# huawei-noah/xingtian

Measured on NVIDIA H100. Metric: learner env-steps/sec (Atari 84x84x4 PPO), higher is better.
Workload: dtype f32 (bf16x3 split on wgmma, fp32 accumulate in registers)

## Files before the change

### xingtian_b200/csrc/optim.cuh

```cuda
#pragma once
#include <cuda_bf16.h>
#include <cuda_runtime.h>
#include <stdint.h>

#include "bp_gemm.cuh"
#include "launch.cuh"

namespace xtb {

constexpr int OPT_CHUNK = 1024;
constexpr int OPT_THREADS = 256;

struct AdamState {
  float beta1_pow, beta2_pow, lr_t, grad_norm;
  unsigned int iterations;
};
struct AdamHyper {
  float lr, beta1, beta2, eps, clip;
  float decay;
};

__device__ __forceinline__ void adam_prep(AdamState* st, const AdamHyper* hyp, double* norm_sq, float* seg_scale, int n_seg,
                                          int clip_mode, float grad_scale) {
  const float clip = hyp->clip, beta1 = hyp->beta1, beta2 = hyp->beta2;
  float lr = hyp->lr;
  if (hyp->decay != 0.f) lr = lr / (1.f + hyp->decay * (float)st->iterations);
  st->iterations += 1;
  double tot = 0.0;
  for (int s = 0; s < n_seg; s++) tot += norm_sq[s];
  float gs = fabsf(grad_scale);
  float gnorm = (float)sqrt(tot) * gs;
  st->grad_norm = gnorm;
  if (clip_mode == 1) {
    float sc = clip / fmaxf(gnorm, clip);
    for (int s = 0; s < n_seg; s++) seg_scale[s] = sc * grad_scale;
  } else if (clip_mode == 2) {
    for (int s = 0; s < n_seg; s++) {
      float n = (float)sqrt(norm_sq[s]) * gs;
      seg_scale[s] = (n > clip ? clip / n : 1.f) * grad_scale;
    }
  } else {
    for (int s = 0; s < n_seg; s++) seg_scale[s] = grad_scale;
  }
  for (int s = 0; s < n_seg; s++) norm_sq[s] = 0.0;
  float b1p = st->beta1_pow * beta1, b2p = st->beta2_pow * beta2;
  st->beta1_pow = b1p; st->beta2_pow = b2p;
  st->lr_t = lr * sqrtf(1.f - b2p) / (1.f - b1p);
}

constexpr int SQN_GROUP = 4;
__global__ void __launch_bounds__(OPT_THREADS)
sqnorm_kernel(const float* __restrict__ g, const int* __restrict__ blk_seg,
              const long long* __restrict__ blk_beg, const int* __restrict__ blk_len, int n_blk,
              double* __restrict__ norm_sq, unsigned int* __restrict__ ticket, AdamState* st, const AdamHyper* __restrict__ hyp,
              float* seg_scale, int n_seg, int clip_mode, float grad_scale) {
  pdl_wait(); pdl_trigger();
  __shared__ float red[OPT_THREADS / 32];
  auto flush = [&](float s, int seg) {
#pragma unroll
    for (int o = 16; o > 0; o >>= 1) s += __shfl_xor_sync(0xffffffffu, s, o);
    if ((threadIdx.x & 31) == 0) red[threadIdx.x >> 5] = s;
    __syncthreads();
    if (threadIdx.x < 32) {
      float t = threadIdx.x < OPT_THREADS / 32 ? red[threadIdx.x] : 0.f;
#pragma unroll
      for (int o = 16; o > 0; o >>= 1) t += __shfl_xor_sync(0xffffffffu, t, o);
      if (threadIdx.x == 0) atomicAdd(norm_sq + seg, (double)t);
    }
    __syncthreads();
  };
  const int e0 = blockIdx.x * SQN_GROUP, e1 = min(e0 + SQN_GROUP, n_blk);
  float s = 0.f;
  int cur = blk_seg[e0];
  for (int e = e0; e < e1; e++) {
    if (blk_seg[e] != cur) { flush(s, cur); s = 0.f; cur = blk_seg[e]; }
    const float* p = g + blk_beg[e];
    const int n = blk_len[e];
    if ((blk_beg[e] & 3) == 0) {
      const int nv = n & ~3;
      for (int i = threadIdx.x * 4; i < nv; i += OPT_THREADS * 4) {
        const float4 v = *reinterpret_cast<const float4*>(p + i);
        s = fmaf(v.x, v.x, s); s = fmaf(v.y, v.y, s); s = fmaf(v.z, v.z, s); s = fmaf(v.w, v.w, s);
      }
      for (int i = nv + threadIdx.x; i < n; i += OPT_THREADS) { float v = p[i]; s = fmaf(v, v, s); }
    } else {
      for (int i = threadIdx.x; i < n; i += OPT_THREADS) { float v = p[i]; s = fmaf(v, v, s); }
    }
  }
  flush(s, cur);
  if (threadIdx.x == 0) {
    __threadfence();
    if (atomicAdd(ticket, 1u) == gridDim.x - 1) {
      __threadfence();
      *ticket = 0;
      adam_prep(st, hyp, norm_sq, seg_scale, n_seg, clip_mode, grad_scale);
    }
  }
}

__global__ void __launch_bounds__(OPT_THREADS)
adam_kernel(float* __restrict__ p, const float* __restrict__ g, float* __restrict__ m,
            float* __restrict__ v, const int* __restrict__ blk_seg,
            const long long* __restrict__ blk_beg, const int* __restrict__ blk_len,
            const float* __restrict__ seg_scale, const AdamState* __restrict__ st, const AdamHyper* __restrict__ hyp,
            const bp::BlobSeg* __restrict__ bsegs, int n_bsegs, __nv_bfloat16* __restrict__ w_hi, long long w_lo_off) {
  pdl_wait(); pdl_trigger();
  const float beta1 = hyp->beta1, beta2 = hyp->beta2, eps = hyp->eps;
  long long beg = blk_beg[blockIdx.x];
  int n = blk_len[blockIdx.x];
  float sc = seg_scale[blk_seg[blockIdx.x]];
  float lr_t = st->lr_t;
  const bool vec = ((beg & 3) == 0);
  int nv = vec ? (n & ~3) : 0;
  for (int i = threadIdx.x * 4; i < nv; i += OPT_THREADS * 4) {
    long long j = beg + i;
    float4 g4 = *reinterpret_cast<const float4*>(g + j);
    float4 m4 = *reinterpret_cast<const float4*>(m + j);
    float4 v4 = *reinterpret_cast<const float4*>(v + j);
    float4 p4 = *reinterpret_cast<const float4*>(p + j);
    float gg[4] = {g4.x * sc, g4.y * sc, g4.z * sc, g4.w * sc};
    float mm[4] = {m4.x, m4.y, m4.z, m4.w}, vv[4] = {v4.x, v4.y, v4.z, v4.w}, pp[4] = {p4.x, p4.y, p4.z, p4.w};
#pragma unroll
    for (int q = 0; q < 4; q++) {
      mm[q] = beta1 * mm[q] + (1.f - beta1) * gg[q];
      vv[q] = beta2 * vv[q] + (1.f - beta2) * gg[q] * gg[q];
      pp[q] -= lr_t * mm[q] / (sqrtf(vv[q]) + eps);
    }
    *reinterpret_cast<float4*>(m + j) = make_float4(mm[0], mm[1], mm[2], mm[3]);
    *reinterpret_cast<float4*>(v + j) = make_float4(vv[0], vv[1], vv[2], vv[3]);
    *reinterpret_cast<float4*>(p + j) = make_float4(pp[0], pp[1], pp[2], pp[3]);
    if (w_hi) bp::blob_store4(bsegs, n_bsegs, w_hi, w_lo_off, j, pp);
  }
  for (int i = nv + threadIdx.x; i < n; i += OPT_THREADS) {
    long long j = beg + i;
    float gg = g[j] * sc;
    float mm = beta1 * m[j] + (1.f - beta1) * gg;
    float vv = beta2 * v[j] + (1.f - beta2) * gg * gg;
    m[j] = mm; v[j] = vv;
    float pn = p[j] - lr_t * mm / (sqrtf(vv) + eps);
    p[j] = pn;
    if (w_hi) bp::blob_store1(bsegs, n_bsegs, w_hi, w_lo_off, j, pn);
  }
}

template <bool CENTRED>
__global__ void __launch_bounds__(OPT_THREADS)
rmsprop_kernel(float* __restrict__ p, const float* __restrict__ g, float* __restrict__ ms, float* __restrict__ mg,
               const int* __restrict__ blk_seg, const long long* __restrict__ blk_beg, const int* __restrict__ blk_len,
               const float* __restrict__ seg_scale, const AdamHyper* __restrict__ hyp, float rho, float rms_eps,
               const bp::BlobSeg* __restrict__ bsegs, int n_bsegs, __nv_bfloat16* __restrict__ w_hi, long long w_lo_off) {
  pdl_wait(); pdl_trigger();
  const long long beg = blk_beg[blockIdx.x];
  const int n = blk_len[blockIdx.x];
  const float sc = seg_scale[blk_seg[blockIdx.x]], lr = hyp->lr;
  const bool vec = ((beg & 3) == 0);
  const int nv = vec ? (n & ~3) : 0;
  for (int i = threadIdx.x * 4; i < nv; i += OPT_THREADS * 4) {
    const long long j = beg + i;
    const float4 g4 = *reinterpret_cast<const float4*>(g + j);
    const float4 s4 = *reinterpret_cast<const float4*>(ms + j);
    const float4 a4 = CENTRED ? *reinterpret_cast<const float4*>(mg + j) : make_float4(0.f, 0.f, 0.f, 0.f);
    const float4 p4 = *reinterpret_cast<const float4*>(p + j);
    float gg[4] = {g4.x * sc, g4.y * sc, g4.z * sc, g4.w * sc};
    float ss[4] = {s4.x, s4.y, s4.z, s4.w}, aa[4] = {a4.x, a4.y, a4.z, a4.w}, pp[4] = {p4.x, p4.y, p4.z, p4.w};
#pragma unroll
    for (int q = 0; q < 4; q++) {
      ss[q] = rho * ss[q] + (1.f - rho) * gg[q] * gg[q];
      if (CENTRED) {
        aa[q] = rho * aa[q] + (1.f - rho) * gg[q];
        pp[q] -= lr * gg[q] / sqrtf(ss[q] - aa[q] * aa[q] + rms_eps);
      } else {
        pp[q] -= lr * gg[q] / sqrtf(ss[q] + rms_eps);
      }
    }
    *reinterpret_cast<float4*>(ms + j) = make_float4(ss[0], ss[1], ss[2], ss[3]);
    if (CENTRED) *reinterpret_cast<float4*>(mg + j) = make_float4(aa[0], aa[1], aa[2], aa[3]);
    *reinterpret_cast<float4*>(p + j) = make_float4(pp[0], pp[1], pp[2], pp[3]);
    if (w_hi) bp::blob_store4(bsegs, n_bsegs, w_hi, w_lo_off, j, pp);
  }
  for (int i = nv + threadIdx.x; i < n; i += OPT_THREADS) {
    const long long j = beg + i;
    const float gg = g[j] * sc;
    const float ss = rho * ms[j] + (1.f - rho) * gg * gg;
    ms[j] = ss;
    float pn;
    if (CENTRED) {
      const float aa = rho * mg[j] + (1.f - rho) * gg;
      mg[j] = aa;
      pn = p[j] - lr * gg / sqrtf(ss - aa * aa + rms_eps);
    } else {
      pn = p[j] - lr * gg / sqrtf(ss + rms_eps);
    }
    p[j] = pn;
    if (w_hi) bp::blob_store1(bsegs, n_bsegs, w_hi, w_lo_off, j, pn);
  }
}

}
```

### xingtian_b200/csrc/xtb_engine.cu

```cuda
#include "../../include/xtb200.h"

#include <cuda_runtime.h>

#include <atomic>
#include <cmath>
#include <cstdarg>
#include <cstdio>
#include <cstring>
#include <map>
#include <memory>
#include <string>
#include <tuple>
#include <vector>

#include "gemm_f32.cuh"
#include "optim.cuh"
#include "rl_kernels.cuh"
#include "qmix.cuh"
#include "scc.cuh"
#include "stager.cuh"
#include "bp_gemm.cuh"
#include "comm.cuh"
#include <cstdlib>
#include <type_traits>
// ... 1320 lines not shown
      rc = comm_fork_allreduce(comm, net->grads + early_off, early_cnt, st);
      if (rc) return rc;
    }
    if (lp.d.kind == XTB_DUELING) {
      const int s = lp.d.src, s2 = lp.d.k;
      rc = op_dgrad(net, i, written[s] ? 1 : 0, batch, st, false, written[s2] ? 1 : 0);
      if (rc) return rc;
      written[s] = written[s2] = 1; has_grad[s] = has_grad[s2] = 1;
    } else if (lp.d.src != 0) {
      int s = lp.d.src;
      rc = op_dgrad(net, i, written[s] ? 1 : 0, batch, st, fuse_bias[s] == 1);
      if (rc) return rc;
      written[s] = 1; has_grad[s] = 1; dy[s] = 1;
    }
  }
  if (o.dobs) {
    bool first = true;
    for (int i = 0; i < nl; i++) {
      const LayerPlan& lp = net->L[i];
      if (lp.d.src != 0 || lp.d.kind != XTB_DENSE || (o.skip & (1u << i))) continue;
      if (!has_grad[i + 1]) continue;
      int rc = ensure_f32(net, i + 1, batch, true, st);
      if (rc) return rc;
      ADense<float> al{(const float*)gout_f32(net, i + 1), nullptr, lp.N};
      BTransposed bl{net->params + lp.w_off, lp.N};
      EpiDgrad ep{o.dobs, o.dobs, 0, lp.K, first ? 0 : 1, nullptr, 0};
      launch_gemm(al, bl, ep, batch, lp.K, lp.N, false, st);
      LAUNCH_CHECK();
      first = false;
    }
    if (first) CUDA_TRY(cudaMemsetAsync(o.dobs, 0, (size_t)batch * net->tsize[0] * sizeof(float), st));
  }
  int rc = flush_reductions(net, st);
  if (rc || !comm || comm->world == 1) return rc;
  if (early_cnt == 0) return xtb_comm_allreduce(comm, net->grads, net->n_params, stream);
  int nrc = g_nccl.GroupStart();
  if (!nrc && early_off > 0) nrc = g_nccl.AllReduce(net->grads, net->grads, (size_t)early_off, kNcclFloat, kNcclSum, comm->comm, st);
  const long long tail = net->n_params - (early_off + early_cnt);
  if (!nrc && tail > 0)
    nrc = g_nccl.AllReduce(net->grads + early_off + early_cnt, net->grads + early_off + early_cnt, (size_t)tail, kNcclFloat, kNcclSum, comm->comm, st);
  int erc = g_nccl.GroupEnd();
  if (nrc || erc) return fail(XTB_ERR_CUDA, "ncclAllReduce: %s", g_nccl.GetErrorString(nrc ? nrc : erc));
  return comm_join(comm, st);
}

extern "C" int xtb_net_bench_layer(xtb_net* net, int layer, int which, const void* obs, const int32_t* gather_idx,
                                   int batch, void* stream) {
  if (!net || !net->ws || !net->grads) return fail(XTB_ERR_STATE, "xtb_net_bench_layer: net not bound");
  if (layer < 0 || layer >= (int)net->L.size() || batch <= 0 || batch > net->max_batch) return fail(XTB_ERR_ARG, "bad layer/batch");
  cudaStream_t st = S(stream);
  for (int t = 1; t <= (int)net->L.size(); t++)
    for (bool grad : {false, true})
      if (forms(net, t, grad) == kNone) wrote(net, t, grad, kF32);
  if (which == 0) return op_forward(net, layer, net->params, true, obs, gather_idx, batch, batch, false, st);
  if (which == 1) { int rc = op_wgrad(net, layer, obs, gather_idx, batch, st, true); net->pending.clear(); return rc; }
  if (which == 2) {
    if (net->L[layer].d.src == 0) return fail(XTB_ERR_ARG, "layer reads the observation: no data gradient");
    int rc = op_dgrad(net, layer, 0, batch, st);
    net->pending.clear();
    return rc;
  }
  if (which == 3) { wrote(net, 0, false, kNone); return op_decode(net, obs, gather_idx, batch, st); }
  return fail(XTB_ERR_ARG, "xtb_net_bench_layer: which must be 0..3");
}


extern "C" int xtb_categorical_sample(const float* logits, int batch, int adim, const float* uniforms,
                                      uint64_t seed, uint64_t offset, int32_t* action, float* logp, void* stream) {
  if (!logits || !action || !logp || batch <= 0 || adim <= 0) return fail(XTB_ERR_ARG, "xtb_categorical_sample: bad argument");
  XLAUNCH(sample_kernel<Categorical>, (batch + 127) / 128, 128, 0, S(stream), logits, (const float*)nullptr, batch, batch, adim,
          uniforms, seed, offset, (const unsigned long long*)nullptr, 0, action, logp, (const float*)nullptr, (float*)nullptr);
  LAUNCH_CHECK();
  return XTB_OK;
}

extern "C" int xtb_argmax(const float* q, int batch, int adim, int32_t* action, void* stream) {
  if (!q || !action || batch <= 0 || adim <= 0) return fail(XTB_ERR_ARG, "xtb_argmax: bad argument");
  XLAUNCH(argmax_kernel, (batch + 127) / 128, 128, 0, S(stream), q, batch, adim, action);
  LAUNCH_CHECK();
  return XTB_OK;
}

extern "C" int xtb_gae(const float* value, const float* reward, const uint8_t* done, int n_env, int n_step,
                       float gamma, float lam, int sign_clip, float* adv, float* old_value, float* target_value,
                       void* stream) {
  if (!value || !reward || !done || !adv || !old_value || !target_value) return fail(XTB_ERR_ARG, "xtb_gae: null pointer");
  if (n_env == 0 || n_step == 0) return XTB_OK;
  if (n_env < 0 || n_step < 0) return fail(XTB_ERR_ARG, "xtb_gae: negative size");
  int threads = 128;
  int blocks = (n_env * 32 + threads - 1) / threads;
  XLAUNCH(gae_kernel, blocks, threads, 0, S(stream), value, reward, done, n_env, n_step, gamma, lam, sign_clip, adv,
                                                old_value, target_value);
  LAUNCH_CHECK();
  return XTB_OK;
}

extern "C" int xtb_ppo_loss_grad(const float* logits, const float* v, const int32_t* gather_idx,
                                 const int32_t* action, const float* old_logp, const float* adv,
                                 const float* old_v, const float* target_v, int batch, int adim,
                                 const xtb_ppo_hyper* hp, float inv_count, float* dlogits, float* dv,
                                 float* loss_out, void* stream) {
  if (!logits || !v || !action || !old_logp || !adv || !old_v || !target_v || !hp || !dlogits || !dv || !loss_out)
    return fail(XTB_ERR_ARG, "xtb_ppo_loss_grad: null pointer");
  if (batch <= 0 || adim <= 0 || adim > MAX_ADIM) return fail(XTB_ERR_ARG, "xtb_ppo_loss_grad: batch/adim out of range");
  PpoHyperDev h{hp->clip_ratio, hp->ent_coef, hp->vf_clip, hp->critic_coef};
  XLAUNCH(ppo_loss_kernel, (batch + 127) / 128, 128, 0, S(stream), logits, v, gather_idx, action, old_logp, adv, old_v,
                                                              target_v, batch, adim, h, inv_count, dlogits, dv, loss_out);
  LAUNCH_CHECK();
  return XTB_OK;
}

extern "C" int xtb_diag_gaussian_sample(const float* mean, const float* log_std, int batch, int adim, const float* normals,
                                        uint64_t seed, uint64_t offset, float* action, float* logp, void* stream) {
  if (!mean || !log_std || !action || !logp || batch <= 0 || adim <= 0 || adim > MAX_ADIM)
    return fail(XTB_ERR_ARG, "xtb_diag_gaussian_sample: bad argument");
  XLAUNCH(sample_kernel<DiagGaussian>, (batch + 127) / 128, 128, 0, S(stream), mean, log_std, batch, batch, adim, normals, seed,
          offset, (const unsigned long long*)nullptr, 0, action, logp, (const float*)nullptr, (float*)nullptr);
  LAUNCH_CHECK();
  return XTB_OK;
}

extern "C" int xtb_ppo_gauss_loss_grad(const float* mean, const float* v, const float* log_std, const int32_t* gather_idx,
                                       const float* action, const float* old_logp, const float* adv, const float* old_v,
                                       const float* target_v, int batch, int adim, const xtb_ppo_hyper* hp, float inv_count,
                                       float* dmean, float* dv, float* dlog_std, float* loss_out, void* stream) {
  if (!mean || !v || !log_std || !action || !old_logp || !adv || !old_v || !target_v || !hp || !dmean || !dv || !dlog_std || !loss_out)
    return fail(XTB_ERR_ARG, "xtb_ppo_gauss_loss_grad: null pointer");
  if (batch <= 0 || adim <= 0 || adim > MAX_ADIM) return fail(XTB_ERR_ARG, "xtb_ppo_gauss_loss_grad: batch/adim out of range");
  PpoHyperDev h{hp->clip_ratio, hp->ent_coef, hp->vf_clip, hp->critic_coef};
  if (adim <= 8)
    XLAUNCH(ppo_gauss_loss_kernel<8>, 1, GAUSS_LOSS_THREADS, 0, S(stream), mean, v, log_std, gather_idx, action, old_logp, adv, old_v,
            target_v, batch, adim, h, inv_count, dmean, dv, dlog_std, loss_out);
  else
    XLAUNCH(ppo_gauss_loss_kernel<MAX_ADIM>, 1, GAUSS_LOSS_THREADS, 0, S(stream), mean, v, log_std, gather_idx, action, old_logp, adv,
            old_v, target_v, batch, adim, h, inv_count, dmean, dv, dlog_std, loss_out);
  LAUNCH_CHECK();
  return XTB_OK;
}

extern "C" int xtb_vtrace_loss_grad(const float* tp_logits, const float* baseline, const float* bp_logits,
                                    const int32_t* action, const uint8_t* done, const float* reward,
                                    int n_traj, int step_len, int adim, float gamma, float* dlogits,
                                    float* dbaseline, float* vs_out, float* pg_adv_out, float* loss_out,
                                    void* stream) {
  if (!tp_logits || !baseline || !bp_logits || !action || !done || !reward || !dlogits || !dbaseline || !loss_out)
    return fail(XTB_ERR_ARG, "xtb_vtrace_loss_grad: null pointer");
  if (n_traj <= 0 || step_len < 2 || adim <= 0 || adim > MAX_ADIM) return fail(XTB_ERR_ARG, "xtb_vtrace_loss_grad: bad sizes");
  int threads = 128;
  int blocks = (n_traj * 32 + threads - 1) / threads;
  XLAUNCH(vtrace_kernel, blocks, threads, 0, S(stream), tp_logits, baseline, bp_logits, action, done, reward, n_traj,
                                                   step_len, adim, gamma, dlogits, dbaseline, vs_out, pg_adv_out, loss_out);
  LAUNCH_CHECK();
  return XTB_OK;
}

extern "C" int xtb_dqn_td_loss_grad(const float* q, const float* q_next_target, const float* q_next_online, const int32_t* idx,
                                    const int32_t* action, const float* reward, const uint8_t* done, const float* disc, int batch,
                                    int adim, float gamma, float huber_delta, float inv_count, float* dq, float* y_out,
                                    float* loss_out, void* stream) {
  if (!q || !q_next_target || !action || !reward || !done || !dq || !loss_out) return fail(XTB_ERR_ARG, "xtb_dqn_td_loss_grad: null pointer");
  if (batch <= 0 || adim <= 0) return fail(XTB_ERR_ARG, "xtb_dqn_td_loss_grad: bad sizes");
  XLAUNCH(dqn_loss_kernel, (batch + 127) / 128, 128, 0, S(stream), q, q_next_target, q_next_online, idx, action, reward, done, disc,
          batch, adim, gamma, huber_delta, inv_count, dq, y_out, loss_out);
  LAUNCH_CHECK();
  return XTB_OK;
}
extern "C" int xtb_dqn_loss_grad(const float* q, const float* q_next_target, const float* q_next_online,
                                 const int32_t* action, const float* reward, const uint8_t* done, int batch,
                                 int adim, float gamma, float inv_count, float* dq, float* y_out,
                                 float* loss_out, void* stream) {
  return xtb_dqn_td_loss_grad(q, q_next_target, q_next_online, nullptr, action, reward, done, nullptr, batch, adim, gamma, 0.f,
                              inv_count, dq, y_out, loss_out, stream);
}
extern "C" int xtb_nstep_returns(const float* reward, const uint8_t* done, int n_env, int n_step, int n, float gamma, float* ret,
                                 float* disc, int32_t* last, uint8_t* done_n, void* stream) {
  if (!reward || !done || !ret || !disc || !last || !done_n) return fail(XTB_ERR_ARG, "xtb_nstep_returns: null pointer");
  if (n_env <= 0 || n_step <= 0 || n <= 0) return fail(XTB_ERR_ARG, "xtb_nstep_returns: bad sizes");
  XLAUNCH(nstep_kernel, (n_env * n_step + 127) / 128, 128, 0, S(stream), reward, done, n_env, n_step, n, gamma, ret, disc, last, done_n);
  LAUNCH_CHECK();
  return XTB_OK;
}

extern "C" int xtb_softmax(const float* logits, int batch, int adim, float* probs, void* stream) {
  if (!logits || !probs || batch <= 0 || adim <= 0) return fail(XTB_ERR_ARG, "xtb_softmax: bad argument");
  XLAUNCH(softmax_rows_kernel, (batch + 127) / 128, 128, 0, S(stream), logits, batch, adim, probs);
  LAUNCH_CHECK();
  return XTB_OK;
}

extern "C" int xtb_impala_keras_loss_grad(const float* logits, const float* v, const int32_t* idx, const float* action_mat,
                                          const float* adv, const float* target_v, int batch, int adim, float ent_coef,
                                          float value_weight, float loss_scale, float* dlogits, float* dv, float* loss_out,
                                          void* stream) {
  if (!logits || !v || !action_mat || !adv || !target_v || !dlogits || !dv || !loss_out)
    return fail(XTB_ERR_ARG, "xtb_impala_keras_loss_grad: null pointer");
  if (batch <= 0 || adim <= 0 || adim > MAX_ADIM) return fail(XTB_ERR_ARG, "xtb_impala_keras_loss_grad: batch/adim out of range");
  XLAUNCH(impala_keras_loss_kernel, 1, KERAS_LOSS_THREADS, 0, S(stream), logits, v, idx, action_mat, adv, target_v, batch, adim,
          ent_coef, value_weight, loss_scale, dlogits, dv, loss_out);
  LAUNCH_CHECK();
  return XTB_OK;
}

extern "C" int xtb_mse_loss_grad(const float* q, const float* y, int batch, int adim, float inv_count, float* dq,
                                 float* loss_out, void* stream) {
  if (!q || !y || !dq || !loss_out || batch <= 0 || adim <= 0) return fail(XTB_ERR_ARG, "xtb_mse_loss_grad: bad argument");
  long long n = (long long)batch * adim;
  XLAUNCH(mse_loss_kernel, (unsigned)((n + 127) / 128), 128, 0, S(stream), q, y, n, inv_count, dq, loss_out);
  LAUNCH_CHECK();
  return XTB_OK;
}

struct xtb_adam {
  long long count = 0;
  float lr, beta1, beta2, eps, clip;
  int clip_mode = 0, n_seg = 0, n_blk = 0;
  float *m = nullptr, *v = nullptr;
  float* mg = nullptr; float rms_rho = 0.f, rms_eps = 0.f;
  bool rms_plain = false;
  int* blk_seg = nullptr; long long* blk_beg = nullptr; int* blk_len = nullptr;
  double* norm_sq = nullptr; float* seg_scale = nullptr; AdamState* st = nullptr; AdamHyper* hyp = nullptr; unsigned int* ticket = nullptr;
  void* buf = nullptr;
};

static inline bool misaligned16(const void* p) { return (uintptr_t)p % 16 != 0; }

extern "C" int xtb_adam_create(long long count, float lr, float beta1, float beta2, float eps, int clip_mode,
                               float clip, const long long* seg_offsets, int n_seg, float* m, float* v,
                               xtb_adam** out) {
  if (count <= 0 || !m || !v || !out) return fail(XTB_ERR_ARG, "xtb_adam_create: bad argument");
  if (clip_mode != XTB_CLIP_NONE && clip_mode != XTB_CLIP_GLOBAL_NORM && clip_mode != XTB_CLIP_PER_TENSOR)
    return fail(XTB_ERR_ARG, "xtb_adam_create: unknown clip_mode %d", clip_mode);
  if (clip_mode != XTB_CLIP_NONE && !(clip > 0.f))
    return fail(XTB_ERR_ARG, "xtb_adam_create: clip must be > 0 with a clipping mode (got %g)", (double)clip);
  if (misaligned16(m) || misaligned16(v)) return fail(XTB_ERR_ARG, "xtb_adam_create: m and v must be 16-byte aligned");
  std::vector<long long> seg;
  if (clip_mode == XTB_CLIP_PER_TENSOR) {
    if (!seg_offsets || n_seg <= 0) return fail(XTB_ERR_ARG, "per-tensor clip needs segment offsets");
    seg.assign(seg_offsets, seg_offsets + n_seg + 1);
    if (seg.front() != 0 || seg.back() != count) return fail(XTB_ERR_ARG, "segment offsets must span [0,count]");
    for (int s = 0; s < n_seg; s++)
      if (seg[s + 1] < seg[s])
        return fail(XTB_ERR_ARG, "xtb_adam_create: segment offsets must not decrease (offset %d: %lld < %lld)", s + 1, seg[s + 1], seg[s]);
  } else {
    seg = {0, count};
  }
  auto* o = new xtb_adam();
  o->count = count; o->lr = lr; o->beta1 = beta1; o->beta2 = beta2; o->eps = eps; o->clip = clip;
  o->clip_mode = clip_mode; o->n_seg = (int)seg.size() - 1; o->m = m; o->v = v;
  std::vector<int> bseg, blen; std::vector<long long> bbeg;
  for (int s = 0; s < o->n_seg; s++)
    for (long long b = seg[s]; b < seg[s + 1]; b += OPT_CHUNK) {
      bseg.push_back(s); bbeg.push_back(b); blen.push_back((int)std::min<long long>(OPT_CHUNK, seg[s + 1] - b));
    }
  o->n_blk = (int)bseg.size();
  AdamState init{1.f, 1.f, 0.f, 0.f, 0u};
  AdamHyper hy{lr, beta1, beta2, eps, clip, 0.f};
  cudaError_t e = cudaMemset(m, 0, count * sizeof(float));
  if (e == cudaSuccess) e = cudaMemset(v, 0, count * sizeof(float));
  if (e != cudaSuccess) { delete o; return fail(XTB_ERR_CUDA, "xtb_adam_create: %s", cudaGetErrorString(e)); }
  if (int rc = carve_scratch("xtb_adam_create", &o->buf, {{&o->blk_seg, o->n_blk, bseg.data()}, {&o->blk_beg, o->n_blk, bbeg.data()},
                                                          {&o->blk_len, o->n_blk, blen.data()}, {&o->norm_sq, o->n_seg},
                                                          {&o->seg_scale, o->n_seg}, {&o->st, 1, &init}, {&o->hyp, 1, &hy},
                                                          {&o->ticket, 1}})) {
    delete o;
    return rc;
  }
  *out = o;
  return XTB_OK;
}

extern "C" void xtb_adam_destroy(xtb_adam* o) {
  if (!o) return;
  drop_graphs_of(o);
  cudaDeviceSynchronize();
  cudaFree(o->buf);
  delete o;
}

static int adam_step_impl(xtb_adam* o, float* params, const float* grads, float grad_scale, void* stream, xtb_net* net);
extern "C" int xtb_adam_step(xtb_adam* o, float* params, const float* grads, float grad_scale, void* stream) {
  return adam_step_impl(o, params, grads, grad_scale, stream, nullptr);
}
extern "C" int xtb_adam_step_net(xtb_adam* o, xtb_net* net, float grad_scale, void* stream) {
  if (!net || !net->ws || !net->params || !net->grads) return fail(XTB_ERR_STATE, "xtb_adam_step_net: net not bound");
  if (!o || o->count != net->n_params) return fail(XTB_ERR_ARG, "xtb_adam_step_net: optimiser/net size mismatch");
  return adam_step_impl(o, net->params, net->grads, grad_scale, stream, net);
}
static int adam_step_impl(xtb_adam* o, float* params, const float* grads, float grad_scale, void* stream, xtb_net* net) {
  if (!o || !params || !grads) return fail(XTB_ERR_ARG, "xtb_adam_step: null pointer");
  if (misaligned16(params) || misaligned16(grads) || misaligned16(o->m) || misaligned16(o->v) || misaligned16(o->mg))
    return fail(XTB_ERR_ARG, "xtb_adam_step: params, grads and the optimiser slots must be 16-byte aligned");
  cudaStream_t st = S(stream);
  XLAUNCH(sqnorm_kernel, (o->n_blk + SQN_GROUP - 1) / SQN_GROUP, OPT_THREADS, 0, st, grads, o->blk_seg, o->blk_beg, o->blk_len, o->n_blk, o->norm_sq, o->ticket, o->st,
          (const AdamHyper*)o->hyp, o->seg_scale, o->n_seg, o->clip_mode, grad_scale);
  LAUNCH_CHECK();
  const bool blobs = net && !net->blob_segs.empty();
  if (o->mg || o->rms_plain) {
    XLAUNCH(o->mg ? rmsprop_kernel<true> : rmsprop_kernel<false>, o->n_blk, OPT_THREADS, 0, st, params, grads, o->m, o->mg, o->blk_seg, o->blk_beg, o->blk_len,
            o->seg_scale, (const AdamHyper*)o->hyp, o->rms_rho, o->rms_eps, blobs ? (const bp::BlobSeg*)(net->ws + net->segs_off) : nullptr,
            blobs ? (int)net->blob_segs.size() : 0, blobs ? (__nv_bfloat16*)(net->ws + net->blob_off) : nullptr, blobs ? net->blob_elems : 0LL);
    LAUNCH_CHECK();
    return XTB_OK;
  }
  XLAUNCH(adam_kernel, o->n_blk, OPT_THREADS, 0, st, params, grads, o->m, o->v, o->blk_seg, o->blk_beg, o->blk_len,
          o->seg_scale, o->st, (const AdamHyper*)o->hyp, blobs ? (const bp::BlobSeg*)(net->ws + net->segs_off) : nullptr,
          blobs ? (int)net->blob_segs.size() : 0, blobs ? (__nv_bfloat16*)(net->ws + net->blob_off) : nullptr, blobs ? net->blob_elems : 0LL);
  LAUNCH_CHECK();
  return XTB_OK;
}

extern "C" const float* xtb_adam_grad_norm(const xtb_adam* o) { return o ? &o->st->grad_norm : nullptr; }
extern "C" int xtb_opt_use_rmsprop(xtb_adam* o, float* mean_grad, float decay, float epsilon) {
  if (!o || !mean_grad) return fail(XTB_ERR_ARG, "xtb_opt_use_rmsprop: null pointer");
  if (misaligned16(mean_grad)) return fail(XTB_ERR_ARG, "xtb_opt_use_rmsprop: mean_grad must be 16-byte aligned");
  if (!(decay > 0.f && decay < 1.f) || !(epsilon > 0.f)) return fail(XTB_ERR_ARG, "xtb_opt_use_rmsprop: decay in (0,1), epsilon > 0");
  drop_graphs_of(o);
  {
    std::vector<float> ones((size_t)o->count, 1.f);
    CUDA_TRY(cudaDeviceSynchronize());
    CUDA_TRY(cudaMemcpy(o->m, ones.data(), ones.size() * sizeof(float), cudaMemcpyHostToDevice));
    CUDA_TRY(cudaMemset(mean_grad, 0, ones.size() * sizeof(float)));
  }
  o->mg = mean_grad; o->rms_rho = decay; o->rms_eps = epsilon; o->rms_plain = false;
  return XTB_OK;
}
extern "C" int xtb_opt_use_rmsprop_plain(xtb_adam* o, float decay, float epsilon) {
  if (!o) return fail(XTB_ERR_ARG, "xtb_opt_use_rmsprop_plain: null pointer");
  if (!(decay > 0.f && decay < 1.f) || !(epsilon > 0.f)) return fail(XTB_ERR_ARG, "xtb_opt_use_rmsprop_plain: decay in (0,1), epsilon > 0");
  drop_graphs_of(o);
  {
    std::vector<float> ones((size_t)o->count, 1.f);
    CUDA_TRY(cudaDeviceSynchronize());
    CUDA_TRY(cudaMemcpy(o->m, ones.data(), ones.size() * sizeof(float), cudaMemcpyHostToDevice));
  }
  o->mg = nullptr; o->rms_rho = decay; o->rms_eps = epsilon; o->rms_plain = true;
  return XTB_OK;
}
extern "C" int xtb_adam_set_lr(xtb_adam* o, float lr) {
  if (!o) return fail(XTB_ERR_ARG, "null optimiser");
  o->lr = lr;
  CUDA_TRY(cudaDeviceSynchronize());
  CUDA_TRY(cudaMemcpy(&o->hyp->lr, &lr, sizeof lr, cudaMemcpyHostToDevice));
  return XTB_OK;
}
extern "C" int xtb_adam_set_decay(xtb_adam* o, float decay) {
  if (!o) return fail(XTB_ERR_ARG, "null optimiser");
  if (!(decay >= 0.f)) return fail(XTB_ERR_ARG, "xtb_adam_set_decay: decay must be >= 0");
  CUDA_TRY(cudaDeviceSynchronize());
  CUDA_TRY(cudaMemcpy(&o->hyp->decay, &decay, sizeof decay, cudaMemcpyHostToDevice));
  return XTB_OK;
}

struct EngineStream { cudaStream_t st = nullptr; cudaEvent_t in = nullptr, out = nullptr; };
static EngineStream g_engine_streams[64];
struct StreamScope {
  cudaStream_t st = nullptr;
  EngineStream* es = nullptr;
  int begin(void* stream, bool side_if_null) {
    st = S(stream);
    if (st || !side_if_null) return XTB_OK;
    int dev = 0;
    CUDA_TRY(cudaGetDevice(&dev));
    if (dev < 0 || dev >= 64) return fail(XTB_ERR_ARG, "device index %d out of range", dev);
    EngineStream& e = g_engine_streams[dev];
    if (!e.st) {
      CUDA_TRY(cudaStreamCreateWithFlags(&e.st, cudaStreamNonBlocking));
      CUDA_TRY(cudaEventCreateWithFlags(&e.in, cudaEventDisableTiming));
      CUDA_TRY(cudaEventCreateWithFlags(&e.out, cudaEventDisableTiming));
    }
    CUDA_TRY(cudaEventRecord(e.in, nullptr));
    CUDA_TRY(cudaStreamWaitEvent(e.st, e.in, 0));
    es = &e; st = e.st;
    return XTB_OK;
  }
  int end() {
    if (!es) return XTB_OK;
    CUDA_TRY(cudaEventRecord(es->out, es->st));
    CUDA_TRY(cudaStreamWaitEvent(nullptr, es->out, 0));
    es = nullptr;
    return XTB_OK;
  }
};
static int g_fuse_heads = [] { const char* e = getenv("XTB_FUSE_HEADS"); return e ? atoi(e) : 1; }();
extern "C" int xtb_set_fuse_heads(int on) { g_fuse_heads = on; return XTB_OK; }

enum GraphTag { kPpoTrain = 1, kImpalaTrain, kDqnTrain, kRolloutInfer, kImpalaKerasFit, kImpalaKerasTrain, kMuzeroTrain,
                kMuzeroInitInfer, kMuzeroRecurInfer, kMuzeroSearch, kQmixTrain, kQmixInfer,
                kSccTrain, kSccInfer, kSccCritic };
struct CaptureKey {
  uint64_t tag;
  const void* own[6];
  uint64_t mode[2];
  uint64_t arg[21];
  bool operator<(const CaptureKey& o) const { return memcmp(this, &o, sizeof(CaptureKey)) < 0; }
};
template <class T> static uint64_t key_word(T v) {
  if constexpr (std::is_same_v<T, float>) { uint32_t u; memcpy(&u, &v, sizeof u); return u; }
  else if constexpr (std::is_same_v<T, double>) { uint64_t u; memcpy(&u, &v, sizeof u); return u; }
  else if constexpr (std::is_pointer_v<T>) return (uint64_t)(uintptr_t)v;
  else return (uint64_t)v;
}
template <size_t N, class... A>
static CaptureKey capture_key(GraphTag tag, const void* const (&owners)[N], A... args) {
  static_assert(N < sizeof(CaptureKey::own) / sizeof(void*), "CaptureKey::own too small");
  static_assert(sizeof...(A) <= sizeof(CaptureKey::arg) / sizeof(uint64_t), "CaptureKey::arg too small");
  CaptureKey k;
  memset(&k, 0, sizeof k);
  k.tag = tag;
  std::copy(owners, owners + N, k.own);
  const uint64_t w[] = {key_word(args)...};
  memcpy(k.arg, w, sizeof w);
  return k;
}
struct GraphVal { cudaGraphExec_t exec; long long kernels; };
static constexpr size_t kMaxCachedGraphs = 256;
static std::map<CaptureKey, GraphVal> g_graphs;
static std::atomic<long long> g_graph_replays{0};
extern "C" long long xtb_graph_replay_count(void) { return g_graph_replays.load(); }

static void drop_graphs_of(const void* obj) {
  for (auto it = g_graphs.begin(); it != g_graphs.end();) {
    const auto& own = it->first.own;
    if (std::find(std::begin(own), std::end(own), obj) != std::end(own)) { cudaGraphExecDestroy(it->second.exec); it = g_graphs.erase(it); } else ++it;
  }
}

template <class F>
static int run_graph(CaptureKey key, int use_graph, void* stream, F&& launch) {
  if (!use_graph) return launch(stream);
  key.own[5] = g_comm; key.mode[0] = g_tc_mode; key.mode[1] = g_fuse_heads;
  StreamScope sc;
  int src = sc.begin(stream, true);
  if (src) return src;
  auto it = g_graphs.find(key);
  if (it == g_graphs.end()) {
    cudaStream_t st = sc.st;
    long long before = g_launches.load();
    CUDA_TRY(cudaStreamBeginCapture(st, cudaStreamCaptureModeThreadLocal));
    int rc = launch((void*)st);
    cudaGraph_t graph = nullptr;
    cudaError_t e = cudaStreamEndCapture(st, &graph);
    long long captured = g_launches.load() - before;
    g_launches.store(before);
    if (rc) { if (graph) cudaGraphDestroy(graph); return rc; }
    if (e != cudaSuccess) return fail(XTB_ERR_CUDA, "graph capture failed: %s", cudaGetErrorString(e));
    cudaGraphExec_t exec = nullptr;
    e = cudaGraphInstantiate(&exec, graph, 0);
    cudaGraphDestroy(graph);
    if (e != cudaSuccess) return fail(XTB_ERR_CUDA, "graph instantiate failed: %s", cudaGetErrorString(e));
    if (g_graphs.size() >= kMaxCachedGraphs) {
      for (auto& kv : g_graphs) cudaGraphExecDestroy(kv.second.exec);
      g_graphs.clear();
    }
    it = g_graphs.emplace(key, GraphVal{exec, captured}).first;
  }
  CUDA_TRY(cudaGraphLaunch(it->second.exec, sc.st));
  g_launches.fetch_add(it->second.kernels, std::memory_order_relaxed);
  g_graph_replays.fetch_add(1, std::memory_order_relaxed);
  return sc.end();
}

template <class STEP>
static int ppo_epoch_loop(xtb_net* net, xtb_adam* opt, int N, int B, int E, const int32_t* perm, float* loss_per_step,
                          void* stream, STEP&& minibatch) {
  int steps_per_epoch = (N + B - 1) / B;
  CUDA_TRY(cudaMemsetAsync(loss_per_step, 0, sizeof(float) * E * steps_per_epoch, S(stream)));
  int step = 0;
  for (int e = 0; e < E; e++) {
    for (int s0 = 0; s0 < N; s0 += B, step++) {
      int mb = std::min(B, N - s0);
      int rc = minibatch(perm + (long long)e * N + s0, mb, loss_per_step + step);
      if (rc) return rc;
      rc = xtb_adam_step_net(opt, net, 1.f, stream);
      if (rc) return rc;
    }
  }
  return XTB_OK;
}

static float dp_inv_world() { return g_comm ? 1.f / g_comm->world : 1.f; }

static int learner_check(const char* fn, bool missing, const xtb_net* net, const xtb_adam* opt, long long rows, bool dp_ok,
                         long long max_rows = 0, long long n_params = 0) {
  if (missing) return fail(XTB_ERR_ARG, "%s: null pointer", fn);
  if (!net->ws || !net->grads) return fail(XTB_ERR_STATE, "%s: net not bound", fn);
  if (!dp_ok && g_comm) return fail(XTB_ERR_STATE, "%s: data-parallel training (communicator) is not supported", fn);
  if (opt && opt->count != (n_params ? n_params : net->n_params))
    return fail(XTB_ERR_ARG, "%s: optimiser/net size mismatch (%lld != %lld)", fn, opt->count, n_params ? n_params : net->n_params);
  if (!max_rows) max_rows = net->max_batch;
  if (rows < 1 || rows > max_rows) return fail(XTB_ERR_ARG, "%s: batch %lld not in [1, %lld]", fn, rows, max_rows);
  return XTB_OK;
}

static bool ppo_heads_fusable(const xtb_net* net, int pi_t, int v_t, bool infer) {
  const LayerPlan& lpi = net->L[pi_t - 1];
  const LayerPlan& lv = net->L[v_t - 1];
  return g_fuse_heads && lpi.d.kind == XTB_DENSE && lv.d.kind == XTB_DENSE && lpi.d.act == 0 && lv.d.act == 0 &&
         lpi.d.src != 0 && lv.d.src != 0 && lpi.K == lv.K && heads_fit(lpi.K, net->tsize[pi_t], infer);
}

template <class LOSS>
static int heads_fused(xtb_net* net, const void* obs, PpoHeadsArgs& a, int mb, int pi_t, int v_t, unsigned skip,
                       long long ls_off, float* loss_dst, void* stream) {
  const LayerPlan& lpi = net->L[pi_t - 1];
  const LayerPlan& lv = net->L[v_t - 1];
  const int adim = net->tsize[pi_t];
  const int32_t* idx = a.idx;
  CUDA_TRY(cudaMemsetAsync(net->grads, 0, net->n_params * sizeof(float), S(stream)));
  net->pending.clear();
  a.h_pi = out_f32(net, lpi.d.src); a.h_v = out_f32(net, lv.d.src);
  a.g_pi = gout_f32(net, lpi.d.src); a.g_v = gout_f32(net, lv.d.src);
  const bool ext_pi = act_is_ext(lpi.src_act), ext_v = act_is_ext(lv.src_act);
  const bool bp_pi = use_tc(net->L[lpi.d.src - 1]) && net->plane_elems[lpi.d.src] > 0 && !ext_pi;
  const bool bp_v = use_tc(net->L[lv.d.src - 1]) && net->plane_elems[lv.d.src] > 0 && !ext_v;
  a.gp_hi = bp_pi ? gout_bp(net, lpi.d.src).hi : nullptr; a.gp_lo = net->plane_elems[lpi.d.src];
  a.gv_hi = bp_v ? gout_bp(net, lv.d.src).hi : nullptr; a.gv_lo = net->plane_elems[lv.d.src];
  a.pitch = net->pitch;
  a.w_pi = net->params + lpi.w_off; a.b_pi = net->params + lpi.b_off; a.w_v = net->params + lv.w_off; a.b_v = net->params + lv.b_off;
  auto only_feeds_heads = [&](int tsr) { for (int j = 0; j < (int)net->L.size(); j++) if (reads(net->L[j], tsr) && !(skip & (1u << j))) return false; return true; };
  bool bh_pi_ok = net->L[lpi.d.src - 1].d.kind == XTB_DENSE && only_feeds_heads(lpi.d.src) && !ext_pi;
  bool bh_v_ok = net->L[lv.d.src - 1].d.kind == XTB_DENSE && only_feeds_heads(lv.d.src) && !ext_v;
  a.B = mb; a.K = lpi.K; a.A = adim; a.act_pi = dgrad_act(lpi); a.act_v = dgrad_act(lv); a.shared = lpi.d.src == lv.d.src ? 1 : 0;
  int blocks = std::max(1, std::min(kSMs, (mb + 7) / 8));
  const int HK = lpi.K, nacc = HK * adim + 3 * HK + adim + 2 + (LOSS::kLogStd ? adim : 0);
  a.part = (float*)(net->ws + net->heads_part_off); a.slab = (nacc + 3) & ~3;
  size_t shb = (size_t)8 * nacc * sizeof(float);
  { cudaError_t ea = ensure_kernel_attrs(); if (ea != cudaSuccess) return fail(XTB_ERR_CUDA, "kernel attributes: %s", cudaGetErrorString(ea)); }
  XLAUNCH(heads_pick(kHeadsKernels<LOSS>, a.K, a.A)->kern, blocks, 256, shb, S(stream), a);
  LAUNCH_CHECK();
  {
    auto seg = [&](int off, int count, long long dst_off, float* dst_ptr = nullptr) {
      queue_reduction(net, a.part + off, blocks, a.slab, count, dst_off, dst_ptr);
    };
    seg(0, HK * adim, lpi.w_off);
    seg(HK * adim, HK, lv.w_off);
    if (bh_pi_ok) seg(HK * adim + HK, HK, net->L[lpi.d.src - 1].b_off);
    if (!a.shared && bh_v_ok) seg(HK * adim + 2 * HK, HK, net->L[lv.d.src - 1].b_off);
    seg(HK * adim + 3 * HK, adim, lpi.b_off);
    seg(HK * adim + 3 * HK + adim, 1, lv.b_off);
    seg(HK * adim + 3 * HK + adim + 1, 1, 0, loss_dst);
    if (LOSS::kLogStd) seg(HK * adim + 3 * HK + adim + 2, adim, ls_off);
  }
  const int32_t srcs[2] = {lpi.d.src, lv.d.src};
  BackwardOpts o(srcs, a.shared ? 1 : 2);
  o.heads_bp = (bp_pi ? (1u << lpi.d.src) : 0u) | (bp_v ? (1u << lv.d.src) : 0u);
  o.heads_dy = (ext_pi ? (1u << lpi.d.src) : 0u) | (ext_v ? (1u << lv.d.src) : 0u);
  o.bias_done = (bh_pi_ok ? (1u << lpi.d.src) : 0u) | ((lpi.d.src != lv.d.src && bh_v_ok) ? (1u << lv.d.src) : 0u);
  o.skip = skip; o.zero_grads = false; o.all_reduce = true;
  return net_backward_impl(net, obs, idx, mb, stream, o);
}

template <class DIST>
static int ppo_train_launch(xtb_net* net, xtb_adam* opt, const xtb_ppo_rollout* ro, int N, int B, int E, const int32_t* perm,
                            const xtb_ppo_hyper* hp, int pi_t, int v_t, int ls_t, float* loss_per_step, float inv_world,
                            void* stream) {
  const int32_t heads[2] = {pi_t, v_t};
  const auto* action = static_cast<const typename DIST::Action*>(ro->action);
  const int adim = net->tsize[pi_t];
  const long long ls_off = DIST::kLogStd ? net->L[ls_t - 1].w_off : -1;
  const LayerPlan& lpi = net->L[pi_t - 1];
  const LayerPlan& lv = net->L[v_t - 1];
  const bool fuse = ppo_heads_fusable(net, pi_t, v_t, false);
  const unsigned skip = fuse ? ((1u << (pi_t - 1)) | (1u << (v_t - 1))) : 0u;
  return ppo_epoch_loop(net, opt, N, B, E, perm, loss_per_step, stream, [&](const int32_t* idx, int mb, float* step_loss) -> int {
    const unsigned want = fuse ? ((1u << lpi.d.src) | (1u << lv.d.src)) : ((1u << pi_t) | (1u << v_t));
    int rc = net_forward_impl(net, nullptr, ro->obs, idx, mb, stream, skip, want);
    if (rc) return rc;
    if (fuse) {
      PpoHeadsArgs a;
      memset(&a, 0, sizeof a);
      a.idx = idx; a.old_logp = ro->old_logp; a.adv = ro->adv; a.old_v = ro->old_v; a.target_v = ro->target_v;
      if constexpr (DIST::kLogStd) { a.action_f = action; a.log_std = net->params + ls_off; }
      else a.action = action;
      a.logits_out = xtb_net_tensor(net, pi_t); a.v_out = xtb_net_tensor(net, v_t);
      a.hp = PpoHyperDev{hp->clip_ratio, hp->ent_coef, hp->vf_clip, hp->critic_coef}; a.inv_count = inv_world / mb;
      return heads_fused<typename DIST::Loss>(net, ro->obs, a, mb, pi_t, v_t, skip, ls_off, step_loss, stream);
    }
    if constexpr (DIST::kLogStd) {
      CUDA_TRY(cudaMemsetAsync(net->grads, 0, net->n_params * sizeof(float), S(stream)));
      rc = xtb_ppo_gauss_loss_grad(xtb_net_tensor(net, pi_t), xtb_net_tensor(net, v_t), net->params + ls_off, idx, action,
                                   ro->old_logp, ro->adv, ro->old_v, ro->target_v, mb, adim, hp, inv_world / mb,
                                   xtb_net_tensor_grad(net, pi_t), xtb_net_tensor_grad(net, v_t), net->grads + ls_off, step_loss,
                                   stream);
    } else {
      rc = xtb_ppo_loss_grad(xtb_net_tensor(net, pi_t), xtb_net_tensor(net, v_t), idx, action, ro->old_logp, ro->adv,
                             ro->old_v, ro->target_v, mb, adim, hp, inv_world / mb, xtb_net_tensor_grad(net, pi_t),
                             xtb_net_tensor_grad(net, v_t), step_loss, stream);
    }
    if (rc) return rc;
    BackwardOpts o(heads, 2);
    o.zero_grads = !DIST::kLogStd; o.all_reduce = true;
    return net_backward_impl(net, ro->obs, idx, mb, stream, o);
  });
}

static int ppo_heads_check(const char* fn, const xtb_net* net, int pi_t, int v_t, int ls_t) {
  const int nl = (int)net->L.size();
  if (pi_t < 1 || pi_t > nl || v_t < 1 || v_t > nl || net->tsize[v_t] != 1 || net->tsize[pi_t] > MAX_ADIM || ls_t < 0 ||
      ls_t > nl)
    return fail(XTB_ERR_ARG, "%s: bad head tensors", fn);
  if (!ls_t) return XTB_OK;
  const LayerPlan& ls = net->L[ls_t - 1];
  if (ls.d.kind != XTB_LOGSTD || ls.N != net->tsize[pi_t]) return fail(XTB_ERR_ARG, "%s: tensor %d is not a logstd layer of the mean's width", fn, ls_t);
  return XTB_OK;
}

extern "C" int xtb_ppo_heads_plan(const xtb_net* net, int pi_t, int v_t, int infer, int* kpl, int* amax) {
  const char* fn = "xtb_ppo_heads_plan";
// ... 1078 lines not shown
```

Measured before the change: 288,600.

## Prefetch optimizer state before PDL wait and batch chunks per block

Moves the programmatic-dependent-launch wait in the grad-norm and Adam kernels so that block metadata and the m, v and param tiles are loaded before waiting on the previous kernel. This lets those loads overlap the predecessor's tail. The grad-norm kernel gains a fast path that issues all four chunk loads up front when every chunk is a full aligned 1024-element block. Adam now processes two chunks per block with a min-blocks-per-SM launch bound, which adds register pressure and halves the grid.

New measurement: 288,100, median of 6. No clear change (-0.2%).

```diff
diff --git a/xingtian_b200/csrc/optim.cuh b/xingtian_b200/csrc/optim.cuh
--- a/xingtian_b200/csrc/optim.cuh
+++ b/xingtian_b200/csrc/optim.cuh
@@ -54,7 +54,6 @@
               const long long* __restrict__ blk_beg, const int* __restrict__ blk_len, int n_blk,
               double* __restrict__ norm_sq, unsigned int* __restrict__ ticket, AdamState* st, const AdamHyper* __restrict__ hyp,
               float* seg_scale, int n_seg, int clip_mode, float grad_scale) {
-  pdl_wait(); pdl_trigger();
   __shared__ float red[OPT_THREADS / 32];
   auto flush = [&](float s, int seg) {
 #pragma unroll
@@ -70,9 +69,34 @@
     __syncthreads();
   };
   const int e0 = blockIdx.x * SQN_GROUP, e1 = min(e0 + SQN_GROUP, n_blk);
+  int seg[SQN_GROUP];
+  long long beg[SQN_GROUP];
+  bool whole = true;
+#pragma unroll
+  for (int q = 0; q < SQN_GROUP; q++) {
+    seg[q] = 0; beg[q] = 0;
+    if (e0 + q < e1) {
+      seg[q] = blk_seg[e0 + q]; beg[q] = blk_beg[e0 + q];
+      whole = whole && (beg[q] & 3) == 0 && blk_len[e0 + q] == OPT_CHUNK;
+    }
+  }
+  pdl_wait(); pdl_trigger();
   float s = 0.f;
-  int cur = blk_seg[e0];
-  for (int e = e0; e < e1; e++) {
+  int cur = seg[0];
+  if (whole) {
+    static_assert(OPT_CHUNK == 4 * OPT_THREADS, "a whole chunk is one float4 per thread");
+    float4 x[SQN_GROUP];
+#pragma unroll
+    for (int q = 0; q < SQN_GROUP; q++)
+      if (e0 + q < e1) x[q] = *reinterpret_cast<const float4*>(g + beg[q] + threadIdx.x * 4);
+#pragma unroll
+    for (int q = 0; q < SQN_GROUP; q++) {
+      if (e0 + q >= e1) break;
+      if (seg[q] != cur) { flush(s, cur); s = 0.f; cur = seg[q]; }
+      s = fmaf(x[q].x, x[q].x, s); s = fmaf(x[q].y, x[q].y, s); s = fmaf(x[q].z, x[q].z, s); s = fmaf(x[q].w, x[q].w, s);
+    }
+  }
+  for (int e = whole ? e1 : e0; e < e1; e++) {
     if (blk_seg[e] != cur) { flush(s, cur); s = 0.f; cur = blk_seg[e]; }
     const float* p = g + blk_beg[e];
     const int n = blk_len[e];
@@ -98,48 +122,66 @@
   }
 }
 
-__global__ void __launch_bounds__(OPT_THREADS)
+constexpr int ADAM_GROUP = 2;
+__global__ void __launch_bounds__(OPT_THREADS, 4)
 adam_kernel(float* __restrict__ p, const float* __restrict__ g, float* __restrict__ m,
             float* __restrict__ v, const int* __restrict__ blk_seg,
-            const long long* __restrict__ blk_beg, const int* __restrict__ blk_len,
+            const long long* __restrict__ blk_beg, const int* __restrict__ blk_len, int n_blk,
             const float* __restrict__ seg_scale, const AdamState* __restrict__ st, const AdamHyper* __restrict__ hyp,
             const bp::BlobSeg* __restrict__ bsegs, int n_bsegs, __nv_bfloat16* __restrict__ w_hi, long long w_lo_off) {
+  long long beg[ADAM_GROUP];
+  int n[ADAM_GROUP], seg[ADAM_GROUP], nv[ADAM_GROUP];
+  float4 m0[ADAM_GROUP], v0[ADAM_GROUP], p0[ADAM_GROUP];
+  const int i0 = threadIdx.x * 4;
+#pragma unroll
+  for (int c = 0; c < ADAM_GROUP; c++) {
+    const int e = blockIdx.x * ADAM_GROUP + c;
+    beg[c] = 0; n[c] = 0; seg[c] = 0; nv[c] = 0;
+    m0[c] = v0[c] = p0[c] = make_float4(0.f, 0.f, 0.f, 0.f);
+    if (e >= n_blk) continue;
+    beg[c] = blk_beg[e]; n[c] = blk_len[e]; seg[c] = blk_seg[e];
+    nv[c] = (beg[c] & 3) == 0 ? (n[c] & ~3) : 0;
+    if (i0 < nv[c]) {
+      m0[c] = *reinterpret_cast<const float4*>(m + beg[c] + i0);
+      v0[c] = *reinterpret_cast<const float4*>(v + beg[c] + i0);
+      p0[c] = *reinterpret_cast<const float4*>(p + beg[c] + i0);
+    }
+  }
   pdl_wait(); pdl_trigger();
   const float beta1 = hyp->beta1, beta2 = hyp->beta2, eps = hyp->eps;
-  long long beg = blk_beg[blockIdx.x];
-  int n = blk_len[blockIdx.x];
-  float sc = seg_scale[blk_seg[blockIdx.x]];
-  float lr_t = st->lr_t;
-  const bool vec = ((beg & 3) == 0);
-  int nv = vec ? (n & ~3) : 0;
-  for (int i = threadIdx.x * 4; i < nv; i += OPT_THREADS * 4) {
-    long long j = beg + i;
-    float4 g4 = *reinterpret_cast<const float4*>(g + j);
-    float4 m4 = *reinterpret_cast<const float4*>(m + j);
-    float4 v4 = *reinterpret_cast<const float4*>(v + j);
-    float4 p4 = *reinterpret_cast<const float4*>(p + j);
-    float gg[4] = {g4.x * sc, g4.y * sc, g4.z * sc, g4.w * sc};
-    float mm[4] = {m4.x, m4.y, m4.z, m4.w}, vv[4] = {v4.x, v4.y, v4.z, v4.w}, pp[4] = {p4.x, p4.y, p4.z, p4.w};
-#pragma unroll
-    for (int q = 0; q < 4; q++) {
-      mm[q] = beta1 * mm[q] + (1.f - beta1) * gg[q];
-      vv[q] = beta2 * vv[q] + (1.f - beta2) * gg[q] * gg[q];
-      pp[q] -= lr_t * mm[q] / (sqrtf(vv[q]) + eps);
-    }
-    *reinterpret_cast<float4*>(m + j) = make_float4(mm[0], mm[1], mm[2], mm[3]);
-    *reinterpret_cast<float4*>(v + j) = make_float4(vv[0], vv[1], vv[2], vv[3]);
-    *reinterpret_cast<float4*>(p + j) = make_float4(pp[0], pp[1], pp[2], pp[3]);
-    if (w_hi) bp::blob_store4(bsegs, n_bsegs, w_hi, w_lo_off, j, pp);
-  }
-  for (int i = nv + threadIdx.x; i < n; i += OPT_THREADS) {
-    long long j = beg + i;
-    float gg = g[j] * sc;
-    float mm = beta1 * m[j] + (1.f - beta1) * gg;
-    float vv = beta2 * v[j] + (1.f - beta2) * gg * gg;
-    m[j] = mm; v[j] = vv;
-    float pn = p[j] - lr_t * mm / (sqrtf(vv) + eps);
-    p[j] = pn;
-    if (w_hi) bp::blob_store1(bsegs, n_bsegs, w_hi, w_lo_off, j, pn);
+  const float lr_t = st->lr_t;
+#pragma unroll
+  for (int c = 0; c < ADAM_GROUP; c++) {
+    const float sc = seg_scale[seg[c]];
+    for (int i = i0; i < nv[c]; i += OPT_THREADS * 4) {
+      long long j = beg[c] + i;
+      float4 g4 = *reinterpret_cast<const float4*>(g + j);
+      float4 m4 = i == i0 ? m0[c] : *reinterpret_cast<const float4*>(m + j);
+      float4 v4 = i == i0 ? v0[c] : *reinterpret_cast<const float4*>(v + j);
+      float4 p4 = i == i0 ? p0[c] : *reinterpret_cast<const float4*>(p + j);
+      float gg[4] = {g4.x * sc, g4.y * sc, g4.z * sc, g4.w * sc};
+      float mm[4] = {m4.x, m4.y, m4.z, m4.w}, vv[4] = {v4.x, v4.y, v4.z, v4.w}, pp[4] = {p4.x, p4.y, p4.z, p4.w};
+#pragma unroll
+      for (int q = 0; q < 4; q++) {
+        mm[q] = beta1 * mm[q] + (1.f - beta1) * gg[q];
+        vv[q] = beta2 * vv[q] + (1.f - beta2) * gg[q] * gg[q];
+        pp[q] -= lr_t * mm[q] / (sqrtf(vv[q]) + eps);
+      }
+      *reinterpret_cast<float4*>(m + j) = make_float4(mm[0], mm[1], mm[2], mm[3]);
+      *reinterpret_cast<float4*>(v + j) = make_float4(vv[0], vv[1], vv[2], vv[3]);
+      *reinterpret_cast<float4*>(p + j) = make_float4(pp[0], pp[1], pp[2], pp[3]);
+      if (w_hi) bp::blob_store4(bsegs, n_bsegs, w_hi, w_lo_off, j, pp);
+    }
+    for (int i = nv[c] + threadIdx.x; i < n[c]; i += OPT_THREADS) {
+      long long j = beg[c] + i;
+      float gg = g[j] * sc;
+      float mm = beta1 * m[j] + (1.f - beta1) * gg;
+      float vv = beta2 * v[j] + (1.f - beta2) * gg * gg;
+      m[j] = mm; v[j] = vv;
+      float pn = p[j] - lr_t * mm / (sqrtf(vv) + eps);
+      p[j] = pn;
+      if (w_hi) bp::blob_store1(bsegs, n_bsegs, w_hi, w_lo_off, j, pn);
+    }
   }
 }
 
diff --git a/xingtian_b200/csrc/xtb_engine.cu b/xingtian_b200/csrc/xtb_engine.cu
--- a/xingtian_b200/csrc/xtb_engine.cu
+++ b/xingtian_b200/csrc/xtb_engine.cu
@@ -1646,8 +1646,8 @@
     LAUNCH_CHECK();
     return XTB_OK;
   }
-  XLAUNCH(adam_kernel, o->n_blk, OPT_THREADS, 0, st, params, grads, o->m, o->v, o->blk_seg, o->blk_beg, o->blk_len,
-          o->seg_scale, o->st, (const AdamHyper*)o->hyp, blobs ? (const bp::BlobSeg*)(net->ws + net->segs_off) : nullptr,
+  XLAUNCH(adam_kernel, (o->n_blk + ADAM_GROUP - 1) / ADAM_GROUP, OPT_THREADS, 0, st, params, grads, o->m, o->v, o->blk_seg,
+          o->blk_beg, o->blk_len, o->n_blk, o->seg_scale, o->st, (const AdamHyper*)o->hyp, blobs ? (const bp::BlobSeg*)(net->ws + net->segs_off) : nullptr,
           blobs ? (int)net->blob_segs.size() : 0, blobs ? (__nv_bfloat16*)(net->ws + net->blob_off) : nullptr, blobs ? net->blob_elems : 0LL);
   LAUNCH_CHECK();
   return XTB_OK;
```
